# aGotelli/experimental_gpu_programming_for_a_spectral_numerical_integration

Measured on NVIDIA B200. Metric: rod-integrations/sec (N=16, 4 stages, FP64), higher is better.
Workload: dtype f64

## Files before the change

### experimental_gpu_programming_for_a_spectral_numerical_integration_b200/csrc/sri_fused16_dmma.cuh

```cuda
#pragma once
#include "sri_fused16.cuh"
#include "sri_stage_dmma.cuh"

namespace sri {

#ifndef SRI_DMMA_MINBLOCKS
#define SRI_DMMA_MINBLOCKS 4
#endif
#ifndef SRI_DMMA_THREADS
#define SRI_DMMA_THREADS 128
#endif
constexpr int kDmmaThreads = SRI_DMMA_THREADS;
constexpr double kDmmaGrowthDefault = 4.0;

struct DmmaTables {
    static constexpr int Stx = StageTables::total;
    static constexpr int AS = Stx + 256;
    static constexpr int AT = AS + 256;
    static constexpr int total = AT + 256;
};
constexpr int kDmmaTabDoubles = 768;

struct DmmaScratch {
    static constexpr int kx = 0;
    static constexpr int bs = kx + 128;
    static constexpr int fbs = bs + 80;
    static constexpr int xs = fbs + 80;
    static constexpr int rps = xs + 80;
    static constexpr int lbs = rps + 48;
    static constexpr int gam = lbs + 48;
    static constexpr int ns = gam + 48;
    static constexpr int qnode = ns + 48;
    static constexpr int total = qnode + 64;
};
constexpr size_t kDmmaSmem = (kDmmaTabDoubles + (kDmmaThreads / 32) * DmmaScratch::total) * sizeof(double);

#ifndef SRI_DMMA_VOLATILE
#define SRI_DMMA_VOLATILE
#endif
__device__ __forceinline__ void dmma(double& c0, double& c1, double a, double b) {
    asm SRI_DMMA_VOLATILE("mma.sync.aligned.m8n8k4.row.col.f64.f64.f64.f64 {%0,%1}, {%2}, {%3}, {%0,%1};" : "+d"(c0), "+d"(c1) : "d"(a), "d"(b));
}
__device__ __forceinline__ double dmma_zero(double a, double b) {
    double d0, d1;
    const double z = 0.0;
    asm("mma.sync.aligned.m8n8k4.row.col.f64.f64.f64.f64 {%0,%1}, {%2}, {%3}, {%4,%4};" : "=d"(d0), "=d"(d1) : "d"(a), "d"(b), "d"(z));
    (void)d1;
    return d0;
}
__device__ __forceinline__ double flip_sign(double v, unsigned mask) {
    return __hiloint2double(__double2hiint(v) ^ (int)mask, __double2loint(v));
}

template <int KT0>
__device__ __forceinline__ void stage_dmma16(const double* at, const double* rhs_lane, int lane, double (&acc)[2][2]) {
    acc[0][0] = 0.0; acc[0][1] = 0.0; acc[1][0] = 0.0; acc[1][1] = 0.0;
#pragma unroll
    for (int kt = KT0; kt < 4; ++kt) {
        const double b = rhs_lane[4 * kt];
#pragma unroll
        for (int mt = 0; mt < 2; ++mt) dmma(acc[mt][0], acc[mt][1], at[(mt * 4 + kt) * 32 + lane], b);
    }
}
__device__ __forceinline__ void store_stage(double* out, int M, int rho, int cp, const double (&acc)[2][2]) {
#pragma unroll
    for (int mt = 0; mt < 2; ++mt) {
        const int i = 8 * mt + rho;
        if (i < M) {
            if (cp == 0) { out[i] = acc[mt][0]; out[M + i] = acc[mt][1]; }
            else if (cp == 1) out[2 * M + i] = acc[mt][0];
        }
    }
}

template <int MS>
#ifdef SRI_DMMA_MAXNREG
__global__ void __maxnreg__(SRI_DMMA_MAXNREG) fused16_dmma_kernel(const FusedParams p) {
#else
__global__ void __launch_bounds__(kDmmaThreads, SRI_DMMA_MINBLOCKS) fused16_dmma_kernel(const FusedParams p) {
#endif
    if (p.skip && *p.skip) return;
    extern __shared__ __align__(16) double smem[];
    double* stx = smem;
    double* tabAS = smem + 256;
    double* tabAT = smem + 512;
    const int warp = threadIdx.x >> 5, lane = threadIdx.x & 31;
    double* scr = smem + kDmmaTabDoubles + warp * DmmaScratch::total;
    double* qnode = scr + DmmaScratch::qnode;

    constexpr int kWarps = kDmmaThreads / 32;
    if ((long long)blockIdx.x * kWarps >= p.batch) return;
    for (int i = threadIdx.x; i < kDmmaTabDoubles; i += kDmmaThreads) smem[i] = p.ops[DmmaTables::Stx + i];
    for (int i = lane; i < DmmaScratch::total; i += 32) scr[i] = 0.0;
    __syncthreads();

    const int M = MS ? MS : p.M;
    const int N = M + 1;
    const int rho = lane >> 2, cp = lane & 3;
    const int hi = rho >> 2, rr = rho & 3;
    const int row = lane & 15, half = lane >> 4;

    const int srcU_base = 4 * cp + (lane >> 3);
    const bool odd_col = (rho & 1) != 0;
    const int srcL_base = 16 * hi + 4 * (rr ^ cp);
    const unsigned neg_tab = 0x428Eu;
    const unsigned sgL_mask = ((neg_tab >> (4 * rr + cp)) & 1u) << 31;
    const double dpiv0 = (hi == 0 && rr == cp) ? 1.0 : 0.0;
    const double dpiv1 = (hi == 1 && rr == cp) ? 1.0 : 0.0;
    const unsigned hi_mask = hi ? 0x7fffffffu : 0u;
    const int sp = rho >> 1;
    const int idxN = sp ^ cp;
    const unsigned sgN_mask = ((((neg_tab >> (4 * sp + cp)) & 1u) != 0) != (idxN != 0)) ? 0x80000000u : 0u;
    const int diag_code = (rr == 0) ? (4 * hi + cp) : -1;
    const int offb = (rho < 3 ? rho : 3) * 20 + cp;
    const int offb23 = (rho < 3 ? DmmaScratch::bs + rho * 20 : (rho < 6 ? DmmaScratch::fbs + (rho - 3) * 20 : DmmaScratch::bs + 60)) + cp;

    const long long stride = (long long)gridDim.x * kWarps;
    const long long rod0 = (long long)blockIdx.x * kWarps + warp;

    auto prefetch_K = [&](long long rod_, int slot) {
        double* kb = scr + DmmaScratch::kx + slot * 64;
        if (row < M) {
            const double* s = p.K + rod_ * 3 * N + row;
            if (half == 0) { cp_async8(kb + 16 + row, s); cp_async8(kb + 32 + row, s + N); }
            else cp_async8(kb + 48 + row, s + 2 * N);
        }
        if (lane < 4) {
            if (p.q0) cp_async8(kb + 16 * lane + 15, p.q0 + rod_ * 4 + lane);
            else kb[16 * lane + 15] = (lane == 0) ? 1.0 : 0.0;
        }
    };

    if (rod0 < p.batch) prefetch_K(rod0, 0);
    cp_async_commit();

    int it = 0;
    for (long long rod = rod0; rod < p.batch; rod += stride, ++it) {
        const int cur = it & 1;
        if (row < N) {
            const int c0 = half ? 2 : 0, c1 = half ? 3 : 2;
            for (int c = c0; c < c1; ++c) {
                if (p.fbar && row >= 1) cp_async8(scr + DmmaScratch::fbs + 20 * c + (M - row), p.fbar + (rod * 3 + c) * N + row);
                if (p.lbar && row >= 1) cp_async8(scr + DmmaScratch::lbs + 16 * c + row - 1, p.lbar + (rod * 3 + c) * N + row);
                if (p.Gamma) cp_async8(scr + DmmaScratch::gam + 16 * c + row, p.Gamma + (rod * 3 + c) * N + row);
            }
        }
        if (lane < 3) { if (p.F_tip) cp_async8(scr + DmmaScratch::fbs + 20 * lane + 15, p.F_tip + rod * 3 + lane); }
        else if (lane >= 4 && lane < 7) { if (p.M_tip) cp_async8(scr + DmmaScratch::xs + 20 * (lane - 4) + 15, p.M_tip + rod * 3 + lane - 4); }
        else if (lane >= 8 && lane < 11) { if (p.r0) cp_async8(scr + DmmaScratch::bs + 20 * (lane - 8) + 15, p.r0 + rod * 3 + lane - 8); }
        if (rod + stride < p.batch) prefetch_K(rod + stride, cur ^ 1);
        cp_async_commit();
        cp_async_wait<1>();
        __syncwarp();

        const double* kb = scr + DmmaScratch::kx + cur * 64;
        double c[8][2][2];
        {
            double kq[2][2];
#pragma unroll
            for (int ct = 0; ct < 2; ++ct) {
                const double2 v = *reinterpret_cast<const double2*>(kb + 16 * rr + 8 * ct + 2 * cp);
                kq[ct][0] = v.x; kq[ct][1] = v.y;
            }
#pragma unroll
            for (int t = 0; t < 8; ++t)
#pragma unroll
                for (int ct = 0; ct < 2; ++ct) {
                    const double2 s = *reinterpret_cast<const double2*>(stx + (2 * t + hi) * 16 + 8 * ct + 2 * cp);
#pragma unroll
                    for (int e = 0; e < 2; ++e) {
                        const int dcode = 4 * e + (t - 4 * ct);
                        const bool candidate = (t - 4 * ct >= 0) && (t - 4 * ct < 4) && !(ct == 1 && t == 7 && e == 1);
                        const double d = (candidate && diag_code == dcode) ? 1.0 : 0.0;
                        c[t][ct][e] = fma(e ? s.y : s.x, kq[ct][e], d);
                    }
                }
        }
        bool bad = false;
        const int growth_log = p.growth_log;
        double la[8], un[2];
#pragma unroll
        for (int k = -1; k < 15; ++k) {
            const int kn = k + 1;
            const bool upd = (k >= 0) && (MS != 0 || k < M);
            const bool prep = (kn < 15) && (MS != 0 || kn < M);
            const int nt = (kn >> 1) & 7, nh = kn & 1, nc = (kn >> 3) & 1, ncp = (kn & 7) >> 1, ne = kn & 1;
            if (upd) {
#pragma unroll
                for (int ct = 0; ct < 2; ++ct)
                    if (8 * ct + 7 > k) dmma(c[nt][ct][0], c[nt][ct][1], la[nt], un[ct]);
            }
            double un0[2] = {0.0, 0.0}, r0n = 0.0, t2 = 0.0;
            unsigned mx = 0u;
            int thr = 0;
            if (prep) {
                const int srcU = 16 * nh + srcU_base;
                const double pcs = __shfl_sync(0xffffffffu, c[nt][nc][ne], 16 * nh + 4 * idxN + ncp);
                const double bn0 = flip_sign(pcs, sgN_mask);
#pragma unroll
                for (int ct = nc; ct < 2; ++ct) {
                    const double v0 = __shfl_sync(0xffffffffu, c[nt][ct][0], srcU);
                    const double v1 = __shfl_sync(0xffffffffu, c[nt][ct][1], srcU);
                    un0[ct] = dmma_zero(odd_col ? v1 : v0, bn0);
                }
                const double nu = __shfl_sync(0xffffffffu, un0[nc], 4 * (kn & 7));
                double r0;
                asm("rcp.approx.ftz.f64 %0, %1;" : "=d"(r0) : "d"(nu));
                const double e = fma(-nu, r0, 1.0);
                t2 = fma(e, e, e);
                r0n = flip_sign(r0, 0x80000000u);
                const int hn = __double2hiint(nu);
                thr = (int)(((long long)hn + 0x3ff00000LL + (long long)growth_log) >> 1);
                if (hn < 0x05000000 || hn >= 0x7ff00000) thr = -1;
            }
            const int srcL = srcL_base + ncp;
#pragma unroll
            for (int tt = 0; tt < 8; ++tt) {
                const int t = (nt + tt) & 7;
                if (upd && tt != 0) {
#pragma unroll
                    for (int ct = 0; ct < 2; ++ct)
                        if (8 * ct + 7 > k) dmma(c[t][ct][0], c[t][ct][1], la[t], un[ct]);
                }
                if (prep) {
                    const double v = __shfl_sync(0xffffffffu, c[t][nc][ne], srcL);
                    const unsigned h = (unsigned)__double2hiint(v) & 0x7fffffffu;
                    if (t > nt) mx = max(mx, h);
                    else if (t == nt && nh == 0) mx = max(mx, h & hi_mask);
                    la[t] = flip_sign(v, sgL_mask);
                    if (tt == 0) la[t] -= nh ? dpiv1 : dpiv0;
                }
            }
            if (prep) {
                bad = bad || ((int)mx > thr);
#pragma unroll
                for (int ct = 0; ct < 2; ++ct)
                    if (8 * ct + 7 > kn) {
#ifdef SRI_DMMA_RFOLD
                        un[ct] = un0[ct] * fma(r0n, t2, r0n);
#else
                        const double a = un0[ct] * r0n; un[ct] = fma(a, t2, a);
#endif
                    }
            }
        }
        const bool flagged = __any_sync(0xffffffffu, bad);
        cp_async_wait<0>();
        const bool keep = !(flagged && p.rod_list);
        if (!keep && lane == 0) p.rod_list[atomicAdd(p.rod_count, 1)] = (int)rod;
        if (cp == 3) {
#pragma unroll
            for (int t = 0; t < 8; ++t) qnode[4 * (2 * t + hi) + rr] = c[t][1][1];
        }
        __syncwarp();
        if (lane < 4) qnode[4 * M + lane] = kb[16 * lane + 15];
        if (p.info && keep && lane == 0) p.info[rod] = flagged ? -1 : 0;
        __syncwarp();
        quat q; q.w = 1.0; q.x = 0.0; q.y = 0.0; q.z = 0.0;
        if (row <= M) q = ld_quat(qnode + 4 * row);
        if (p.Q && keep && row < M) {
            double* d = p.Q + rod * 4 * M + (2 * half) * M + row;
            d[0] = half ? q.y : q.w;
            d[M] = half ? q.z : q.x;
        }

        if (p.r || p.n || p.m) {
            double bv0 = 0.0, bv1 = 0.0, bv2 = 0.0;
            if (row <= M) {
                if (p.Gamma) {
                    const double* gm = scr + DmmaScratch::gam + row;
                    q_rotate(q, gm[0], gm[16], gm[32], bv0, bv1, bv2);
                } else {
                    q_rotate_e1(q, bv0, bv1, bv2);
                }
            }
            if (half == 0) {
                double* rp = scr + DmmaScratch::rps + row;
                rp[0] = bv0; rp[16] = bv1; rp[32] = bv2;
                if (row < 15) { double* b = scr + DmmaScratch::bs + row; b[0] = bv0; b[20] = bv1; b[40] = bv2; }
            }
            __syncwarp();
            double acc[2][2];
            stage_dmma16<0>(tabAS, scr + offb23, lane, acc);
#pragma unroll
            for (int mt = 0; mt < 2; ++mt) {
                const int i = 8 * mt + rho;
                if (i < M && keep) {
                    if (p.r) {
                        double* d = p.r + rod * 3 * M + i;
                        if (cp == 0) { d[0] = acc[mt][0]; d[M] = acc[mt][1]; }
                        else if (cp == 1) d[2 * M] = acc[mt][0];
                    }
                    if (p.n) {
                        double* d = p.n + rod * 3 * M + (M - 1 - i);
                        if (cp == 1) d[0] = acc[mt][1];
                        else if (cp == 2) { d[M] = acc[mt][0]; d[2 * M] = acc[mt][1]; }
                    }
                }
            }
            if (p.n || p.m) {
                if (p.m) {
                    double* nsv = scr + DmmaScratch::ns;
#pragma unroll
                    for (int mt = 0; mt < 2; ++mt) {
                        const int i = 8 * mt + rho;
                        if (i < M) {
                            if (cp == 1) nsv[M - 1 - i] = acc[mt][1];
                            else if (cp == 2) { nsv[16 + M - 1 - i] = acc[mt][0]; nsv[32 + M - 1 - i] = acc[mt][1]; }
                        }
                    }
                    __syncwarp();
                    if (half == 0 && row < 15) {
                        const double n0 = nsv[row], n1 = nsv[16 + row], n2 = nsv[32 + row];
                        const double* rp = scr + DmmaScratch::rps + row + 1;
                        const double rp0 = rp[0], rp1 = rp[16], rp2 = rp[32];
                        double l0 = 0.0, l1 = 0.0, l2 = 0.0;
                        if (p.lbar) { const double* lb = scr + DmmaScratch::lbs + row; l0 = lb[0]; l1 = lb[16]; l2 = lb[32]; }
                        double* x = scr + DmmaScratch::xs + row;
                        x[0] = fma(rp1, n2, fma(-rp2, n1, l0));
                        x[20] = fma(rp2, n0, fma(-rp0, n2, l1));
                        x[40] = fma(rp0, n1, fma(-rp1, n0, l2));
                    }
                    __syncwarp();
                    stage_dmma16<0>(tabAT, scr + DmmaScratch::xs + offb, lane, acc);
                    if (keep) store_stage(p.m + rod * 3 * M, M, rho, cp, acc);
                }
            }
        }
        __syncwarp();
    }
    cp_async_wait<0>();
}

}
```

Measured before the change: 229.6 million.

## Replace full Gauss-Jordan elimination with forward elimination plus DMMA back-substitution

The elimination loop now only updates rows below the pivot, dropping the upper-triangle updates of full Gauss-Jordan. Each normalized pivot row is stored to a new per-warp shared-memory block. The solution quaternions are then recovered by a backward substitution pass that also uses DMMA tiles and shuffles. This cuts the tensor-core MMAs and shuffles in the main loop but adds shared-memory traffic, a larger per-warp scratch footprint that may lower occupancy, and a serial back-substitution chain.

New measurement: 267.4 million (median of 6 runs). 1.16x the previous value.

```diff
diff --git a/experimental_gpu_programming_for_a_spectral_numerical_integration_b200/csrc/sri_fused16_dmma.cuh b/experimental_gpu_programming_for_a_spectral_numerical_integration_b200/csrc/sri_fused16_dmma.cuh
--- a/experimental_gpu_programming_for_a_spectral_numerical_integration_b200/csrc/sri_fused16_dmma.cuh
+++ b/experimental_gpu_programming_for_a_spectral_numerical_integration_b200/csrc/sri_fused16_dmma.cuh
@@ -31,8 +31,11 @@
     static constexpr int gam = lbs + 48;
     static constexpr int ns = gam + 48;
     static constexpr int qnode = ns + 48;
-    static constexpr int total = qnode + 64;
+    static constexpr int ust = qnode + 64;
+    static constexpr int total = ust + 740;
 };
+__host__ __device__ constexpr int ucol(int j) { return j < 8 ? 92 * j + 64 : 92 * (j - 8); }
+static_assert(ucol(7) + 32 <= 740, "DmmaScratch::ust size");
 constexpr size_t kDmmaSmem = (kDmmaTabDoubles + (kDmmaThreads / 32) * DmmaScratch::total) * sizeof(double);
 
 #ifndef SRI_DMMA_VOLATILE
@@ -106,12 +109,12 @@
     const unsigned neg_tab = 0x428Eu;
     const unsigned sgL_mask = ((neg_tab >> (4 * rr + cp)) & 1u) << 31;
     const double dpiv0 = (hi == 0 && rr == cp) ? 1.0 : 0.0;
-    const double dpiv1 = (hi == 1 && rr == cp) ? 1.0 : 0.0;
     const unsigned hi_mask = hi ? 0x7fffffffu : 0u;
     const int sp = rho >> 1;
     const int idxN = sp ^ cp;
     const unsigned sgN_mask = ((((neg_tab >> (4 * sp + cp)) & 1u) != 0) != (idxN != 0)) ? 0x80000000u : 0u;
     const int diag_code = (rr == 0) ? (4 * hi + cp) : -1;
+    double* const ustl = scr + DmmaScratch::ust + 92 * rho + cp;
     const int offb = (rho < 3 ? rho : 3) * 20 + cp;
     const int offb23 = (rho < 3 ? DmmaScratch::bs + rho * 20 : (rho < 6 ? DmmaScratch::fbs + (rho - 3) * 20 : DmmaScratch::bs + 60)) + cp;
 
@@ -182,7 +185,7 @@
 #pragma unroll
         for (int k = -1; k < 15; ++k) {
             const int kn = k + 1;
-            const bool upd = (k >= 0) && (MS != 0 || k < M);
+            const bool upd = (k >= 0) && (k < 14) && (MS != 0 || k < M - 1);
             const bool prep = (kn < 15) && (MS != 0 || kn < M);
             const int nt = (kn >> 1) & 7, nh = kn & 1, nc = (kn >> 3) & 1, ncp = (kn & 7) >> 1, ne = kn & 1;
             if (upd) {
@@ -215,20 +218,18 @@
             }
             const int srcL = srcL_base + ncp;
 #pragma unroll
-            for (int tt = 0; tt < 8; ++tt) {
-                const int t = (nt + tt) & 7;
-                if (upd && tt != 0) {
+            for (int t = nt; t < 8; ++t) {
+                if (upd && t != nt) {
 #pragma unroll
                     for (int ct = 0; ct < 2; ++ct)
                         if (8 * ct + 7 > k) dmma(c[t][ct][0], c[t][ct][1], la[t], un[ct]);
                 }
-                if (prep) {
+                if (prep && (t != nt || nh == 0)) {
                     const double v = __shfl_sync(0xffffffffu, c[t][nc][ne], srcL);
                     const unsigned h = (unsigned)__double2hiint(v) & 0x7fffffffu;
-                    if (t > nt) mx = max(mx, h);
-                    else if (t == nt && nh == 0) mx = max(mx, h & hi_mask);
+                    mx = max(mx, t != nt ? h : (h & hi_mask));
                     la[t] = flip_sign(v, sgL_mask);
-                    if (tt == 0) la[t] -= nh ? dpiv1 : dpiv0;
+                    if (t == nt) la[t] -= dpiv0;
                 }
             }
             if (prep) {
@@ -241,17 +242,40 @@
 #else
                         const double a = un0[ct] * r0n; un[ct] = fma(a, t2, a);
 #endif
+                        ustl[(ct ? ucol(8) : ucol(0)) + 4 * kn] = un[ct];
                     }
             }
         }
         const bool flagged = __any_sync(0xffffffffu, bad);
+        __syncwarp();
+        {
+            int ln;
+            asm volatile("mov.u32 %0, %%laneid;" : "=r"(ln));
+            const int qm = ln >> 2, qs = ln & 3;
+            const double* ust = scr + DmmaScratch::ust;
+            double y[2][2];
+#pragma unroll
+            for (int b = 0; b < 2; ++b)
+#pragma unroll
+                for (int e = 0; e < 2; ++e) y[b][e] = qm < 4 ? ust[ucol(15) + 4 * (8 * b + 2 * qs + e) + (qm & 3)] : 0.0;
+            const unsigned sgQ_mask = ((0x284Eu >> (4 * (qm & 3) + qs)) & 1u) << 31;
+            const int srcQ_base = 4 * (qm ^ qs);
+#pragma unroll
+            for (int j = 14; j >= 0; --j) {
+                if (MS != 0 || j < M) {
+                    const int b = j >> 3, n = j & 7;
+                    const double v = __shfl_sync(0xffffffffu, y[b][n & 1], srcQ_base + (n >> 1));
+                    if (qm < 4 && qs == 0) qnode[4 * j + qm] = flip_sign(v, 0x80000000u);
+                    const double a = flip_sign(v, sgQ_mask);
+#pragma unroll
+                    for (int bb = 0; bb <= b; ++bb)
+                        if (8 * bb < j) dmma(y[bb][0], y[bb][1], a, ust[ucol(j) + 32 * bb + ln]);
+                }
+            }
+        }
         cp_async_wait<0>();
         const bool keep = !(flagged && p.rod_list);
         if (!keep && lane == 0) p.rod_list[atomicAdd(p.rod_count, 1)] = (int)rod;
-        if (cp == 3) {
-#pragma unroll
-            for (int t = 0; t < 8; ++t) qnode[4 * (2 * t + hi) + rr] = c[t][1][1];
-        }
         __syncwarp();
         if (lane < 4) qnode[4 * M + lane] = kb[16 * lane + 15];
         if (p.info && keep && lane == 0) p.info[rod] = flagged ? -1 : 0;
```
